# verdurin/pbdagcon

Hardware: AMD Instinct MI355X
Metric: consensus bases/sec (whole node) (higher is better)
Workload: dtype u8

## Files before the change

### pbdagcon_amd/csrc/api_run.hip.h

```cpp
namespace {

#define DQ_KMAX 52u
struct DgPlanIn { uint32_t T; uint64_t n_alns, sum_bb; uint32_t gcuts, max_segments, min_segment_len, seg_env, merge_q; };
struct DgPlan { uint32_t seg_max, seg_min, use_q, bp_max; };
static DgPlan dg_plan_pieces(const DgPlanIn &in) {
    DgPlan pl;
    const uint32_t T = in.T;
    pl.seg_min = in.min_segment_len;
    if (!pl.seg_min) pl.seg_min = (uint32_t)std::min<uint64_t>(768, std::max<uint64_t>(192, in.sum_bb / 8192));
    if (in.max_segments) pl.seg_max = in.max_segments > 64u ? 64u : in.max_segments;
    else if (in.seg_env) pl.seg_max = in.seg_env;
    else if (in.gcuts) pl.seg_max = 64;
    else { uint32_t sm = T ? 8192u / T : 8u; pl.seg_max = sm < 8u ? 8u : sm > 256u ? 256u : sm; }
    if (in.gcuts && !in.min_segment_len) pl.seg_min = 256;
    pl.use_q = 0;
    if (in.merge_q && !in.gcuts && pl.seg_max != 1) {
        const uint32_t slots = 1024u * DQ_WAVES;
        if (in.max_segments || in.seg_env) pl.use_q = 1;
        else if (T && in.n_alns <= (uint64_t)DQ_KMAX * T) {
            const uint64_t avail = std::min<uint64_t>(256, std::max<uint64_t>(1, in.sum_bb / T / 128));
            const uint64_t k = (uint64_t)T * avail / DQ_ROWS / slots;
            if (k >= 1 || (uint64_t)T * avail / DQ_ROWS * 10u >= 6u * slots) {
                const uint64_t sm = std::min<uint64_t>(avail, std::max<uint64_t>(k, 1) * slots * DQ_ROWS / T);
                if (sm >= 2) { pl.seg_max = (uint32_t)sm; pl.use_q = 1; }
// ... 130 lines not shown
    p.q_kmax = c->use_q && !c->opts.max_segments && !c->seg_env && c->max_k > DQ_KMAX ? DQ_KMAX : 0u;
    p.bp_seg_min = (c->seg_min + 2u) / 3u;
    p.seg_max = c->seg_max; p.seg_min = c->seg_min; p.cuts = c->run.cuts.as<uint32_t>(); p.bp_max = c->bp_max; p.cuts_bp = c->run.cuts_bp.as<uint32_t>(); p.bp_stat = c->run.bp_stat.as<float>(); p.bp_len = c->run.bp_len.as<uint32_t>();
    p.gcuts = c->gcuts; p.sh_log = c->sh_log;
    p.rd_s = c->run.rd.as<uint32_t>(); p.rd_e = p.rd_s + c->A; p.rd_lead = p.rd_e + c->A; p.rd_trail = p.rd_lead + c->A;
    p.pro_state = c->run.pro_state.as<uint32_t>(); p.sh_cnt = c->run.sh_cnt.as<uint32_t>();
    p.queue0 = c->run.queue0.as<int32_t>(); p.bp_end = c->run.bp_end.as<uint32_t>(); p.bp_ab = c->run.bp_ab.as<float>();
    p.defer = c->run.defer.as<uint32_t>(); p.cns_tmp0 = c->run.cns_tmp0.as<uint8_t>();
    p.seg_done = c->run.seg_done.as<uint32_t>(); p.wl_first = c->run.wl_first.as<uint32_t>();
    p.worklist = c->run.worklist.as<uint32_t>(); p.worklist_cap = c->worklist_cap;
    p.cns = c->run.cns.as<uint8_t>(); p.cns_cap = c->cns_cap;
    p.cns_off = c->sb.d<uint64_t>(c->sb.o_cns_off); p.cns_len = c->sb.d<uint32_t>(c->sb.o_cns_len);
    p.seg_first = c->sb.d<uint64_t>(c->sb.o_seg_first); p.n_seg = c->sb.d<uint32_t>(c->sb.o_n_seg);
    p.seg_r0 = c->run.seg.as<int32_t>(); p.seg_r1 = p.seg_r0 + seg_stride(c);
    p.seg_cap = c->seg_cap;
    p.st = c->sb.d<DgStatus>(0);
    if (c->opts.flags & DAGCON_FLAG_BASE_SUPPORT) {
        p.sup_tmp = c->run.sup_tmp.as<uint32_t>(); p.sup_tmp0 = c->run.sup_tmp0.as<uint32_t>();
        p.sup_w = c->run.sup.as<uint16_t>(); p.sup_d = p.sup_w + c->cns_cap;
    }
    if (c->opts.flags & DAGCON_FLAG_BASE_POS) {
        p.pos_tmp = c->run.pos_tmp.as<uint32_t>(); p.pos_tmp0 = c->run.pos_tmp0.as<uint32_t>(); p.pos_out = c->run.pos.as<uint32_t>();
    }
    if (c->ed_batch) {
        p.ed_seg = c->run.ed_seg.as<DgEdSeg>(); p.ed_out = c->run.ed_out.as<DgEdit>(); p.ed_cap = c->ed_cap;
        p.ed_top = c->sb.d<unsigned long long>(c->sb.o_ed_top);
        p.ed_t = c->cg.t.as<const uint8_t>(); p.ed_tbase = c->in.ed_tbase.as<const uint64_t>();
        if (c->evid_batch) p.evid = c->run.evid.as<DgEvid>();
    }
}

void launch_normalize(Ctx *c, const DgParams &p, const bool wide) {
    hipStream_t s = c->stream;
    if (c->A == 0) return;
    (void)hipMemsetAsync(c->run.ckpt.p, 0xFF, c->n_ckpt * 4, s);
    hipLaunchKernelGGL((k_norm_chunk<DG_NW, 64, false>), dim3((c->n_chunks + 63) / 64), dim3(64), 0, s, p);
    hipLaunchKernelGGL((k_norm_chunk<DG_NW_BIG, 32, true>), dim3((c->n_chunks + 31) / 32), dim3(32), 0, s, p);
    hipLaunchKernelGGL(k_norm_scan, dim3((c->A + 63) / 64), dim3(64), 0, s, p);
    if (wide) {
        hipLaunchKernelGGL(k_norm_finish2<uint32_t>, dim3((c->n_chunks + 3) / 4), dim3(256), 0, s, p);
        hipLaunchKernelGGL(k_normalize_slow<uint32_t>, dim3((c->A + 63) / 64), dim3(64), 0, s, p);
    } else {
        hipLaunchKernelGGL(k_norm_finish2<uint8_t>, dim3((c->n_chunks + 3) / 4), dim3(256), 0, s, p);
        hipLaunchKernelGGL(k_normalize_slow<uint8_t>, dim3((c->A + 63) / 64), dim3(64), 0, s, p);
    }
}

int launch_all(Ctx *c) {
    int r = ensure_arenas(c);
    if (r != DAGCON_OK) return r;
    DgParams p;
    fill_params(c, p);
    hipStream_t s = c->stream;
    const bool wide = matc_wide(c);
    if (c->poison & 8) {
        for (DevBuf *b : c->run.all())
            if (b->p && b->cap) HIPCHK(c, hipMemsetAsync(b->p, 0xEE, b->cap, s));
        if (c->sb.bytes > c->sb.zero_bytes) HIPCHK(c, hipMemsetAsync(c->sb.d<char>(c->sb.zero_bytes), 0xEE, c->sb.bytes - c->sb.zero_bytes, s));
    }
    HIPCHK(c, hipMemsetAsync(c->sb.dev.p, 0, c->sb.zero_bytes, s));
    if (c->matc_cells) HIPCHK(c, hipMemsetAsync(c->arena.matC.p, 0, matc_bytes(c), s));
    if (c->poison) {
        if ((c->poison & 1) && c->arena.matA.p) { HIPCHK(c, hipMemsetAsync(c->arena.matA.p, 0xEE, c->arena.matA.cap, s)); HIPCHK(c, hipMemsetAsync(c->arena.matD.p, 0xEE, c->arena.matD.cap, s)); }
        if ((c->poison & 2) && c->arena.nodes.p) { HIPCHK(c, hipMemsetAsync(c->arena.nodes.p, 0xEE, c->arena.nodes.cap, s)); HIPCHK(c, hipMemsetAsync(c->arena.pool.p, 0xEE, c->arena.pool.cap, s)); }
        if ((c->poison & 4) && c->arena.score_b.p) HIPCHK(c, hipMemsetAsync(c->arena.score_b.p, 0xEE, c->arena.score_b.cap, s));
        if ((c->poison & 4) && c->arena.norm.p) HIPCHK(c, hipMemsetAsync(c->arena.norm.p, 0xEE, c->arena.norm.cap, s));
    }
    HIPCHK(c, hipEventRecord(c->ev[0], s));
    launch_normalize(c, p, wide);
    HIPCHK(c, hipEventRecord(c->ev[1], s));
    hipLaunchKernelGGL(k_carve, dim3(1), dim3(1024), 0, s, p);
    if (c->T > 0) {
        const uint32_t rows4 = (c->max_tlen + 2 + 4 * DG_LPW - 1) / (4 * DG_LPW);
        if (c->gcuts && c->A > 0) hipLaunchKernelGGL(k_readspan, dim3((c->A + 63) / 64), dim3(64), 0, s, p);
        if (p.emit_scan && wide) hipLaunchKernelGGL(k_gsum<uint32_t>, dim3(c->T, (c->max_tlen + 2 + 255) / 256), dim3(256), 0, s, p);
        else if (p.emit_scan) hipLaunchKernelGGL(k_gsum<uint8_t>, dim3(c->T, (c->max_tlen + 2 + 1023) / 1024), dim3(256), 0, s, p);
        else hipLaunchKernelGGL(k_groups, dim3(c->T, (c->max_tlen + 2 + 31) / 32), dim3(256), 0, s, p);
        hipLaunchKernelGGL(k_gscan, dim3(c->T), dim3(1024), 0, s, p);
        if (c->A > 0) {
            const dim3 eg(c->T, (c->max_k + DG_ERPW - 1) / DG_ERPW, ((c->max_tlen + 2) >> c->emit_shift) + 1);
            if (wide) hipLaunchKernelGGL(k_emit<uint32_t>, eg, dim3(64), 0, s, p);
            else hipLaunchKernelGGL(k_emit<uint8_t>, eg, dim3(64), 0, s, p);
        }
        const size_t lds = (size_t)4 * 2 * (c->max_k + 2) * sizeof(int32_t);
        if (lds > 65536)
            HIPCHK(c, hipFuncSetAttribute((const void *)k_lists, hipFuncAttributeMaxDynamicSharedMemorySize, (int)lds));
        hipLaunchKernelGGL(k_lists, dim3(c->T, rows4), dim3(256), lds, s, p);
    }
    HIPCHK(c, hipEventRecord(c->ev[2], s));
    if (c->T > 0 && !(c->opts.flags & DAGCON_FLAG_STOP_AFTER_BUILD)) {
        if (c->gcuts) {
            HIPCHK(c, hipMemsetAsync(c->run.worklist.p, 0, 16, s));
            HIPCHK(c, hipMemsetAsync(c->run.seg_done.p, 0, (size_t)c->worklist_cap * (DG_SH_MAX + 1) * 4, s));
            hipLaunchKernelGGL(k_merge_pro, dim3(c->T), dim3(64), 0, s, p);
            hipLaunchKernelGGL(k_cuts2, dim3(c->T), dim3(64), 0, s, p);
            hipLaunchKernelGGL(k_merge_list, dim3(c->list_grid), dim3(64), 0, s, p);
            hipLaunchKernelGGL(k_merge_fin, dim3(c->T), dim3(64), 0, s, p);
        } else {
            hipLaunchKernelGGL(k_cuts, dim3(c->T), dim3(64), 0, s, p);
            if (c->use_q) {
                hipLaunchKernelGGL(k_merge_q, dim3((c->T * c->seg_max + DQ_ROWS - 1u) / DQ_ROWS), dim3(64), 0, s, p);
                if (p.q_kmax) hipLaunchKernelGGL(k_merge, dim3(c->T * c->seg_max), dim3(64), 0, s, p);
            } else hipLaunchKernelGGL(k_merge, dim3(c->T * c->seg_max), dim3(64), 0, s, p);
        }
    }
    HIPCHK(c, hipEventRecord(c->ev[3], s));
    if (c->T > 0 && !(c->opts.flags & (DAGCON_FLAG_STOP_AFTER_BUILD | DAGCON_FLAG_STOP_AFTER_MERGE))) {
        const bool sup = (c->opts.flags & DAGCON_FLAG_BASE_SUPPORT) != 0;
        const bool pos = (c->opts.flags & DAGCON_FLAG_BASE_POS) != 0;
#define DG_BP_LAUNCH(K, GRID)                                                                          \
        do {                                                                                           \
            if (sup && pos) hipLaunchKernelGGL((K<true, true>), GRID, dim3(64), 0, s, p);              \
            else if (sup) hipLaunchKernelGGL((K<true, false>), GRID, dim3(64), 0, s, p);               \
            else if (pos) hipLaunchKernelGGL((K<false, true>), GRID, dim3(64), 0, s, p);               \
            else hipLaunchKernelGGL((K<false, false>), GRID, dim3(64), 0, s, p);                       \
        } while (0)
        hipLaunchKernelGGL(k_bp_terms, dim3(c->T, 16), dim3(256), 0, s, p);
        if (c->gcuts) {
            hipLaunchKernelGGL(k_bp_xtree, dim3(c->T), dim3(64), 0, s, p);
            hipLaunchKernelGGL(k_bp_sweep_ab, dim3(c->T * c->bp_max), dim3(64), 0, s, p);
            hipLaunchKernelGGL(k_bp_comb, dim3(c->T), dim3(64), 0, s, p);
            hipLaunchKernelGGL(k_bp_abs, dim3(c->T * c->bp_max), dim3(256), 0, s, p);
            hipLaunchKernelGGL(k_bp_choose, dim3(c->T * c->bp_max), dim3(256), 0, s, p);
            hipLaunchKernelGGL(k_bp_sweep_abs_g, dim3(c->T * c->bp_max), dim3(64), 0, s, p);
            hipLaunchKernelGGL(k_bp_defer, dim3(c->T), dim3(64), 0, s, p);
            DG_BP_LAUNCH(k_bp_walk_g, dim3(c->T * c->bp_max));
        } else {
            if (p.bp_lane) hipLaunchKernelGGL(k_bp_sweep_l, dim3((c->T * c->bp_max + 7u) / 8u), dim3(64), 0, s, p);
            hipLaunchKernelGGL(k_bp_sweep, dim3(c->T * c->bp_max), dim3(64), 0, s, p);
            hipLaunchKernelGGL(k_bp_check, dim3(c->T), dim3(64), 0, s, p);
            if (p.bp_lane) DG_BP_LAUNCH(k_bp_walk_r, dim3((c->T * c->bp_max + 7u) / 8u));
            else DG_BP_LAUNCH(k_bp_walk, dim3(c->T * c->bp_max));
        }
        DG_BP_LAUNCH(k_bp_join, dim3(c->T));
#undef DG_BP_LAUNCH
        if (c->ed_batch) {
            const dim3 eg((uint32_t)((c->seg_cap + 3) / 4));
            hipLaunchKernelGGL(k_ed_scan_seg<false>, eg, dim3(256), 0, s, p);
            hipLaunchKernelGGL(k_ed_scan, dim3(1), dim3(1024), 0, s, p);
            hipLaunchKernelGGL(k_ed_scan_seg<true>, eg, dim3(256), 0, s, p);
            if (c->evid_batch) {
                hipLaunchKernelGGL(k_ev_windows, eg, dim3(256), 0, s, p);
                if (c->A > 0) hipLaunchKernelGGL(k_ev_count, dim3((c->A + 3) / 4), dim3(256), 0, s, p);
                hipLaunchKernelGGL(k_ev_spread, eg, dim3(256), 0, s, p);
            }
        }
    }
    HIPCHK(c, hipEventRecord(c->ev[4], s));
    HIPCHK(c, hipGetLastError());
    return DAGCON_OK;
}

}

extern "C" {

int dagcon_abi_version(void) { return DAGCON_ABI_VERSION; }

void dagcon_default_opts(dagcon_opts *o) {
    if (!o) return;
    memset(o, 0, sizeof *o);
    o->min_cov = 6; o->min_len = 500; o->trim = 50; o->min_weight = -1; o->device = 0; o->flags = 0;
}

const char *dagcon_last_error(const dagcon_ctx *ctx) {
    return ctx ? reinterpret_cast<const Ctx *>(ctx)->err.c_str() : "null context";
}

int dagcon_create(const dagcon_opts *opts, dagcon_ctx **out) {
    if (!opts || !out) return DAGCON_ERR_INVALID_ARG;
// ... 625 lines not shown
```

### pbdagcon_amd/csrc/k_build.hip.h

```cpp
#pragma once
#include <hip/hip_runtime.h>
#include "dagcon_dev.h"
#include "k_norm_run.hip.h"

#define DG_WAVE 64
#ifndef DG_LPW
#define DG_LPW 8u
#endif

__device__ __forceinline__ bool dg_failed(const DgParams &p) {
    return __hip_atomic_load(&p.st->err_flags, __ATOMIC_RELAXED, __HIP_MEMORY_SCOPE_AGENT) != 0;
}
__device__ __forceinline__ void dg_fail(const DgParams &p, uint32_t bit) {
    atomicOr(&p.st->err_flags, bit);
}
__device__ __forceinline__ void dg_fail_target(const DgParams &p, uint32_t t, uint32_t bit) {
    atomicOr(&p.tfail[t], bit);
}
__device__ __forceinline__ bool dg_tskip(const DgParams &p, uint32_t t) {
    return !p.tactive[t] || __hip_atomic_load(&p.tfail[t], __ATOMIC_RELAXED, __HIP_MEMORY_SCOPE_AGENT) != 0;
}
__device__ __forceinline__ bool dg_askip(const DgParams &p, uint32_t a) {
    return !(p.flags & DG_F_A1_ONLY) && __hip_atomic_load(&p.tfail[p.aln_tgt[a]], __ATOMIC_RELAXED, __HIP_MEMORY_SCOPE_AGENT) != 0;
}
// ... 810 lines not shown
                    const uint8_t qb = DG_Q(c), tb = DG_T(c);
                    if (qb == tb) {
                        const uint32_t cur = bidv[j];
                        acell[j] = ((uint32_t)tb << 25) | (prev + 1u);
                        if (f_anc_ok && kacc != 0u && kacc < (1u << 24)) f_key = kacc | ((pos - f_apos) << 24);
                        DG_DEPART(cur);
                        prev = cur; prev_pos = bbpos; fl = DG_EF_BB | DG_EF_OWN;
                    } else {
                        acell[j] = ((uint32_t)tb << 25) | DG_CELL_DEL;
                    }
                    bbpos++;
                    i++;
                }
            }
            if (p.fold) {
                const unsigned long long em = __ballot(f_key != 0u);
                if (em & (em - 1ull)) {
                    uint32_t fn;
                    const uint32_t vic = dg_emit_fold(em, f_key, f_first, pos, ndt, pool, &fn, lane);
                    if (vic | fn) {
                        const uint32_t dv = vic ? 0u : (f_first + 1u) | ((fn - 1u) << 25);
                        if (f_apos >= pos0) s_D[(f_apos - pos0) * 64 + lane] = dv;
                        if (f_apos < pos0 || f_apos == 0u) DG_ECELL(Dm, f_apos) = dv;
                        if (vic) acell[j] = (acell[j] & 0xFE000000u) | DG_CELL_DUP;
                    }
                }
            }
        }
        if (r < K && lane < DG_ERPW) {
#pragma unroll
            for (int j = 0; j < DG_EB; j++) {
                const uint32_t pos = pos0 + j;
                if (pos <= blen && pos >= P0 && pos < P1) {
                    DG_ECELL(Am, pos) = acell[j];
                    const uint32_t dv = s_D[j * 64 + lane];
                    if (pos > 0 || dv) DG_ECELL(Dm, pos) = dv;
                }
            }
            if (exit_val) DG_ECELL(Am, exitpos) = exit_val;
        }
        pos0 += DG_EB;
    }
    {
        const bool ahead = bbpos != DG_EDONE && (fl & DG_EF_OWN);
        uint32_t q = bbpos, nxt = 0;
        bool found = false, pfx_next = false;
        if (ahead) {
            while (i < hi) {
                const uint16_t c = buf[i];
                const uint8_t qb = DG_Q(c), tb = DG_T(c);
                if (qb == tb) { nxt = bid[q]; found = true; break; }
                if (qb == DG_GAP) { q++; i++; continue; }
                if (tb == DG_GAP) {
                    if (p.emit_scan) pfx_next = true; else nxt = gbase[q] + Cm[q];
                    found = true; break;
                }
                i++;
            }
        }
        if (p.emit_scan) {
            for (unsigned long long m = __ballot(pfx_next); m; m = __ballot(pfx_next)) {
                const uint32_t pp = (uint32_t)__builtin_amdgcn_readlane((int)q, __ffsll((long long)m) - 1);
                const uint32_t x = rvalid ? Cm[pp] : 0u;
                const uint32_t e = dg_wave_excl(x, lane);
                if (pfx_next && q == pp) { nxt = gbase[pp] + e; pfx_next = false; }
            }
        }
        if (ahead) {
            if (!found) {
                nxt = bid[exitpos];
                Am[(uint64_t)exitpos * K + r] = prev + 1u;
            }
            const uint32_t pos0 = 0xFFFFFFFFu;
            DG_DEPART(nxt);
        }
    }
#undef DG_EPW
#undef DG_ECELL
#undef DG_DEPART
#undef DG_COLUMN
#undef DG_STAGE
}

__device__ __forceinline__ int dg_lds_find(volatile int32_t *vals, int n, int x, int lane) {
    for (int b = 0; b < n; b += DG_WAVE) {
        int i = b + lane;
        bool hit = (i < n) && (vals[i] == x);
        unsigned long long m = __ballot(hit);
        if (m) return b + (__ffsll((long long)m) - 1);
    }
    return -1;
}

__device__ __forceinline__ uint32_t dg_pool_alloc(const DgParams &p, uint32_t t, uint32_t words, int lane) {
    uint32_t off = 0;
    if (lane == 0) {
        t = (uint32_t)__builtin_amdgcn_readfirstlane((int)t);
        off = atomicAdd(&p.pool_top[t], words);
        if ((uint64_t)off + words > p.pool_size[t]) { dg_fail(p, DG_E_POOL_TGT); p.st->bad_target = t; off = 0xFFFFFFFFu; }
    }
    return (uint32_t)__builtin_amdgcn_readlane((int)off, 0);
}

__device__ __forceinline__ unsigned long long dg_list_row(int32_t val, int32_t extra, int32_t chain, int32_t ulo, int32_t uhi,
                                                          int lane, int32_t &cnt, unsigned long long &cm) {
    cm = __ballot(val == chain);
    const bool uniq = val >= ulo && val < uhi;
    unsigned long long firsts = __ballot(uniq);
    cnt = 1 + extra;
    unsigned long long rem = __ballot(val != 0 && !uniq) & ~cm;
    while (rem) {
        const int first = __ffsll((long long)rem) - 1;
        const int32_t x = __builtin_amdgcn_readlane(val, first);
        const unsigned long long same = __ballot(val == x);
        rem &= ~same;
        if (lane == first) cnt = __popcll(same) + extra;
        firsts |= 1ull << first;
    }
    return firsts;
}

__device__ __forceinline__ void dg_lists_wave(const DgParams &p, uint32_t t, uint32_t pos0, uint32_t blen, uint32_t K,
                                              int lane) {
    const uint32_t npos = min(DG_LPW, blen + 2 - pos0);
    const uint64_t nb = p.node_base[t];
    const uint64_t bv = p.bbv_base[t];
    const uint32_t capb = dg_capb(K);
    const uint32_t fixed0 = 3u * p.t_nins[t];
    uint32_t *pool = p.pool + p.pool_base[t];
#define DG_LPOOL(OFF) (*reinterpret_cast<uint32_t *>(reinterpret_cast<char *>(pool) + (((uint32_t)(OFF)) << 2)))
    const uint32_t qb = pos0 - 1u + (uint32_t)lane;
    const uint32_t bidl = (lane < (int)DG_LPW + 2 && qb <= blen + 1) ? p.bid[bv + qb] : 0u;
    const uint32_t gbl = (lane <= (int)DG_LPW && pos0 + lane <= blen + 1) ? p.gbase[bv + pos0 + lane] : 0u;
    const uint32_t rb = (uint32_t)lane << 2;
    const bool rl = (uint32_t)lane < K;
    const uint32_t *Ar = p.matA + p.mat_base[t] + (uint64_t)pos0 * K, *Dr = p.matD + p.mat_base[t] + (uint64_t)pos0 * K;
#define DG_LROW(R) (rl ? *reinterpret_cast<const uint32_t *>(reinterpret_cast<const char *>(R) + rb) : 0u)
    uint32_t dcell = DG_LROW(Dr), acell = DG_LROW(Ar);
    const uint32_t lpos = pos0 + (uint32_t)lane;
    uint32_t r_lens = 0;
    uint32_t r_cov = 0;
    uint32_t r_out = fixed0 + lpos * 3u * capb, r_in = r_out + 2u * capb;
    uint32_t r_caps = capb | capb << 16;
    uint32_t pi = 0;
    for (; pi < npos; pi++) {
        const uint32_t pos = pos0 + pi;
        const uint32_t dep = dcell, arr = acell;
        if (pi + 1 < npos) {
            Ar += K; Dr += K;
            dcell = DG_LROW(Dr); acell = DG_LROW(Ar);
        }
        const bool mine = (uint32_t)lane == pi;
        const int32_t v1 = __builtin_amdgcn_readlane((int)bidl, pi + 1) + 1;
        uint32_t out_len = 0, in_len = 0;
        if (pos <= blen) {
            const int32_t val = (int32_t)DG_CELL_ID(dep), extra = (int32_t)(dep >> 25);
            const int32_t chain = __builtin_amdgcn_readlane((int)bidl, pi + 2) + 1;
            const int32_t ulo = __builtin_amdgcn_readlane((int)gbl, pi + 1) + 1;
            int32_t cnt;
            unsigned long long cm;
            const unsigned long long firsts = dg_list_row(val, extra, chain, ulo, chain, lane, cnt, cm);
            const uint32_t n = 1u + (uint32_t)__popcll(firsts);
            uint32_t off = fixed0 + pos * 3u * capb;
            if (n > capb) {
                const uint32_t cap = n + 2u;
                off = dg_pool_alloc(p, t, 2u * cap, lane);
                if (off == 0xFFFFFFFFu) break;
                if (mine) { r_out = off; r_caps = (r_caps & 0xFFFF0000u) | cap; }
            }
            const uint32_t idx = 1u + (uint32_t)__popcll(firsts & ((1ull << lane) - 1ull));
            if (lane == 0) { DG_LPOOL(off) = (uint32_t)(chain - 1); DG_LPOOL(off + 1) = (uint32_t)__popcll(cm); }
            if ((firsts >> lane) & 1ull) { DG_LPOOL(off + 2 * idx) = (uint32_t)(val - 1); DG_LPOOL(off + 2 * idx + 1) = (uint32_t)cnt; }
            out_len = n;
        }
        if (pos >= 1) {
            const uint32_t idf = DG_CELL_ID(arr);
            if (pos <= blen) {
                const unsigned long long covered = __ballot(arr != 0u);
                const uint32_t n_cov = (uint32_t)__popcll(covered);
                const uint32_t n_match = (uint32_t)__popcll(__ballot(arr != 0u && idf != DG_CELL_DEL));
                const uint32_t last_base = covered ? DG_CELL_BASE((uint32_t)__builtin_amdgcn_readlane((int)arr, 63 - __clzll((long long)covered))) : 0u;
                if (mine) r_cov = n_cov | n_match << 8 | last_base << 16;
            }
            const int32_t val = (arr != 0u && idf != DG_CELL_DEL && idf != DG_CELL_DUP) ? (int32_t)idf : 0;
            const int32_t chain = __builtin_amdgcn_readlane((int)bidl, pi) + 1;
            const int32_t ulo = __builtin_amdgcn_readlane((int)gbl, pi) + 1;
            int32_t cnt;
            unsigned long long cm;
            const unsigned long long firsts = dg_list_row(val, 0, chain, ulo, v1, lane, cnt, cm);
            const uint32_t n = 1u + (uint32_t)__popcll(firsts);
            uint32_t off = fixed0 + pos * 3u * capb + 2u * capb;
            if (n > capb) {
                const uint32_t cap = n + 2u;
                off = dg_pool_alloc(p, t, cap, lane);
                if (off == 0xFFFFFFFFu) break;
                if (mine) { r_in = off; r_caps = (r_caps & 0xFFFFu) | cap << 16; }
            }
            const uint32_t idx = 1u + (uint32_t)__popcll(firsts & ((1ull << lane) - 1ull));
            if (lane == 0) DG_LPOOL(off) = (uint32_t)(chain - 1);
            if ((firsts >> lane) & 1ull) DG_LPOOL(off + idx) = (uint32_t)(val - 1);
            in_len = n;
        }
        if (mine) r_lens = out_len | in_len << 16;
    }
    const uint32_t v = __shfl_down(bidl, 1);
    if ((uint32_t)lane < pi) {
        const bool inner = lpos >= 1 && lpos <= blen;
        const uint32_t n_cov = r_cov & 0xFFu, n_match = (r_cov >> 8) & 0xFFu;
        uint32_t base;
        if (lpos == 0) base = '^';
        else if (lpos == blen + 1) base = '$';
        else if (n_cov) base = r_cov >> 16;
        else base = p.bb ? p.bb[p.bb_off[t] + (lpos - 1)] : (uint8_t)'N';
        uint4 *rec = reinterpret_cast<uint4 *>(p.nodes + nb + v);
        rec[0] = make_uint4(r_lens, base | DG_NF_BACKBONE << 8,
                            inner ? 1u + n_match : 0u,
                            r_lens >> 16);
        rec[1] = make_uint4(r_out, r_in, r_caps, inner ? lpos : 0u);
        p.cov[bv + lpos] = inner ? (int32_t)n_cov : 0;
    }
#undef DG_LROW
#undef DG_LPOOL
}

__global__ __launch_bounds__(256) void k_lists(DgParams p) {
    extern __shared__ int32_t s_tmp[];
    const uint32_t t = blockIdx.x;
    if (dg_failed(p) || dg_tskip(p, t)) return;
    const int lane = threadIdx.x & 63, wave = threadIdx.x >> 6;
    const uint32_t blen = p.tlen[t];
    const uint32_t K = (uint32_t)(p.aln_begin[t + 1] - p.aln_begin[t]);
    if (K > DG_WAVE) {
    const uint32_t stride = p.max_k + 2;
    volatile int32_t *vals = s_tmp + (size_t)wave * 2 * stride;
    volatile int32_t *cnts = vals + stride;
    const uint64_t nb = p.node_base[t];
    const uint64_t bv = p.bbv_base[t];
    uint32_t *pool = p.pool + p.pool_base[t];
    const uint32_t *Am0 = p.matA + p.mat_base[t], *Dm0 = p.matD + p.mat_base[t];
    const uint32_t capb = dg_capb(K);
    const uint32_t fixed0 = 3u * p.t_nins[t];
    for (uint32_t pi = 0; pi < DG_LPW; pi++) {
    const uint32_t pos = (blockIdx.y * 4 + wave) * DG_LPW + pi;
    if (pos >= blen + 2) return;
    const uint32_t v = p.bid[bv + pos];
    const uint32_t *Am = Am0 + (uint64_t)pos * K;
    const uint32_t *Dm = Dm0 + (uint64_t)pos * K;
    const uint32_t fixed = fixed0 + pos * 3u * capb;
    uint32_t out_off = fixed, in_off = fixed + 2u * capb;
    uint32_t out_cap = capb, in_cap = capb;
    uint32_t out_len = 0, in_len = 0;
    uint32_t n_match = 0, n_cov = 0, last_base = 0;

    for (int dir = 0; dir < 2; dir++) {
        if (dir == 0 && pos == blen + 1) continue;
        if (dir == 1 && pos == 0) continue;
        const uint32_t *row = dir == 0 ? Dm : Am;
        int n = 1;
        int32_t lv = dir == 0 ? (int32_t)p.bid[bv + pos + 1] : (int32_t)p.bid[bv + pos - 1];
        int32_t lc = 0;
        bool in_lds = false;
        for (uint32_t r0 = 0; r0 < K; r0 += DG_WAVE) {
            const uint32_t r = r0 + lane;
            const uint32_t cell = r < K ? row[r] : 0u;
            int32_t val = (int32_t)DG_CELL_ID(cell);
            const int32_t extra = dir == 0 ? (int32_t)(cell >> 25) : 0;
            if (dir == 1) {
                const uint32_t idf = DG_CELL_ID(cell);
                const unsigned long long covered = __ballot(cell != 0u);
                if (pos <= blen) {
                    n_cov += (uint32_t)__popcll(covered);
                    n_match += (uint32_t)__popcll(__ballot(cell != 0u && idf != DG_CELL_DEL));
                    if (covered) last_base = DG_CELL_BASE((uint32_t)__builtin_amdgcn_readlane((int)cell, 63 - __clzll((long long)covered)));
                }
                val = (cell != 0u && idf != DG_CELL_DEL && idf != DG_CELL_DUP) ? (int32_t)idf : 0;
            }
            unsigned long long rem = __ballot(val != 0);
            if (!in_lds) {
                const int32_t chain = __builtin_amdgcn_readlane(lv, 0) + 1;
                const unsigned long long cm = __ballot(val == chain);
                if (lane == 0) lc += __popcll(cm);
                rem &= ~cm;
            }
            while (rem) {
                const int first = __ffsll((long long)rem) - 1;
                const int32_t x = __builtin_amdgcn_readlane(val, first);
                const unsigned long long same = __ballot(val == x);
                rem &= ~same;
                const int c = __popcll(same) + __builtin_amdgcn_readlane(extra, first);
                if (!in_lds) {
                    const unsigned long long hit = __ballot(lane < n && lv == x - 1);
                    if (hit) {
                        if (lane == __ffsll((long long)hit) - 1) lc += c;
                    } else if (n < DG_WAVE) {
                        if (lane == n) { lv = x - 1; lc = c; }
                        n++;
                    } else {
                        vals[lane] = lv; cnts[lane] = lc;
                        in_lds = true;
                    }
                }
                if (in_lds) {
                    const int idx = dg_lds_find(vals, n, x - 1, lane);
                    if (idx >= 0) {
                        if (lane == 0) cnts[idx] += c;
                    } else {
                        if (lane == 0) { vals[n] = x - 1; cnts[n] = c; }
                        n++;
                    }
                }
            }
        }
        if (n > 65000) { if (lane == 0) dg_fail_target(p, t, DG_E_INTERNAL); return; }
        uint32_t off = dir == 0 ? out_off : in_off;
        if ((uint32_t)n > capb) {
            const uint32_t cap = (uint32_t)n + 2u;
            off = dg_pool_alloc(p, t, dir == 0 ? 2u * cap : cap, lane);
            if (off == 0xFFFFFFFFu) return;
            if (dir == 0) { out_off = off; out_cap = cap; } else { in_off = off; in_cap = cap; }
        }
        if (!in_lds) {
            if (lane < n) {
                if (dir == 0) { pool[off + 2 * lane] = (uint32_t)lv; pool[off + 2 * lane + 1] = (uint32_t)lc; }
                else pool[off + lane] = (uint32_t)lv;
            }
        } else {
            for (int i = lane; i < n; i += DG_WAVE) {
                if (dir == 0) { pool[off + 2 * i] = (uint32_t)vals[i]; pool[off + 2 * i + 1] = (uint32_t)cnts[i]; }
                else pool[off + i] = (uint32_t)vals[i];
            }
        }
        if (dir == 0) out_len = (uint32_t)n; else in_len = (uint32_t)n;
    }
    if (lane == 0) {
        const bool inner = pos >= 1 && pos <= blen;
        DgNode nd;
        nd.out_len = (uint16_t)out_len;
        nd.in_len = (uint16_t)in_len;
        nd.flags = DG_NF_BACKBONE; nd.pad = 0;
        if (pos == 0) nd.base = '^';
        else if (pos == blen + 1) nd.base = '$';
        else if (n_cov) nd.base = (uint8_t)last_base;
        else nd.base = p.bb ? p.bb[p.bb_off[t] + (pos - 1)] : (uint8_t)'N';
        nd.weight = inner ? 1 + (int32_t)n_match : 0;
        nd.pending = (int32_t)in_len;
        nd.out_off = out_off; nd.in_off = in_off;
        nd.out_cap = (uint16_t)out_cap; nd.in_cap = (uint16_t)in_cap;
        nd.bbpos = inner ? (int32_t)pos : 0;
        p.cov[bv + pos] = inner ? (int32_t)n_cov : 0;
        p.nodes[nb + v] = nd;
    }
    }
    return;
    }
    const uint32_t pos0 = (blockIdx.y * 4 + (uint32_t)__builtin_amdgcn_readfirstlane(wave)) * DG_LPW;
    if (pos0 < blen + 2) dg_lists_wave(p, t, pos0, blen, K, lane);
}
```

Baseline: 359.7 million.

## Build backbone node lists one position per lane with LDS-staged rows

Replaces the wave-per-position list builder for targets with at most 64 alignments with a new kernel where each lane handles one backbone position. It stages the departure and arrival matrix rows into LDS, dedups them with a small per-lane table of non-unique IDs, and falls back to the old wave-cooperative path only for rows that overflow that table. The goal is to remove the serial per-position loop of ballots and readlanes. The cost is more LDS use, per-lane divergent scans over K cells, and an extra launch, with k_lists now only launched when max_k exceeds 64.

```diff
diff --git a/pbdagcon_amd/csrc/api_run.hip.h b/pbdagcon_amd/csrc/api_run.hip.h
--- a/pbdagcon_amd/csrc/api_run.hip.h
+++ b/pbdagcon_amd/csrc/api_run.hip.h
@@ -236,10 +236,15 @@
             if (wide) hipLaunchKernelGGL(k_emit<uint32_t>, eg, dim3(64), 0, s, p);
             else hipLaunchKernelGGL(k_emit<uint8_t>, eg, dim3(64), 0, s, p);
         }
-        const size_t lds = (size_t)4 * 2 * (c->max_k + 2) * sizeof(int32_t);
-        if (lds > 65536)
-            HIPCHK(c, hipFuncSetAttribute((const void *)k_lists, hipFuncAttributeMaxDynamicSharedMemorySize, (int)lds));
-        hipLaunchKernelGGL(k_lists, dim3(c->T, rows4), dim3(256), lds, s, p);
+        const size_t lds_lanes = (size_t)DG_LL_WAVES * DG_WAVE * (std::min<uint32_t>(c->max_k, DG_WAVE) | 1u) * sizeof(uint32_t);
+        hipLaunchKernelGGL(k_lists_lanes, dim3(c->T, (c->max_tlen + 2 + DG_LL_WAVES * DG_WAVE - 1) / (DG_LL_WAVES * DG_WAVE)),
+                           dim3(DG_LL_WAVES * DG_WAVE), lds_lanes, s, p);
+        if (c->max_k > DG_WAVE) {
+            const size_t lds = (size_t)4 * 2 * (c->max_k + 2) * sizeof(int32_t);
+            if (lds > 65536)
+                HIPCHK(c, hipFuncSetAttribute((const void *)k_lists, hipFuncAttributeMaxDynamicSharedMemorySize, (int)lds));
+            hipLaunchKernelGGL(k_lists, dim3(c->T, rows4), dim3(256), lds, s, p);
+        }
     }
     HIPCHK(c, hipEventRecord(c->ev[2], s));
     if (c->T > 0 && !(c->opts.flags & DAGCON_FLAG_STOP_AFTER_BUILD)) {
diff --git a/pbdagcon_amd/csrc/k_build.hip.h b/pbdagcon_amd/csrc/k_build.hip.h
--- a/pbdagcon_amd/csrc/k_build.hip.h
+++ b/pbdagcon_amd/csrc/k_build.hip.h
@@ -916,6 +916,7 @@
 #undef DG_STAGE
 }
 
+#include "k_lists_row.hip.h"
 __device__ __forceinline__ int dg_lds_find(volatile int32_t *vals, int n, int x, int lane) {
     for (int b = 0; b < n; b += DG_WAVE) {
         int i = b + lane;
@@ -954,107 +955,193 @@
     return firsts;
 }
 
-__device__ __forceinline__ void dg_lists_wave(const DgParams &p, uint32_t t, uint32_t pos0, uint32_t blen, uint32_t K,
+struct DgPosLists { uint32_t o_len, o_off, o_cap, i_len, i_off, i_cap, cov; };
+
+__device__ __forceinline__ bool dg_lists_pos(const DgParams &p, uint32_t t, uint32_t *pool, uint32_t pos, uint32_t blen,
+                                             uint32_t capb, uint32_t fixed0, int lane, bool do_out, bool do_in,
+                                             uint32_t dep, uint32_t arr, int32_t v1, int32_t chain_o, int32_t ulo_o,
+                                             int32_t chain_i, int32_t ulo_i, DgPosLists &r) {
+#define DG_LPOOL(OFF) (*reinterpret_cast<uint32_t *>(reinterpret_cast<char *>(pool) + (((uint32_t)(OFF)) << 2)))
+    if (do_out) {
+        const int32_t val = (int32_t)DG_CELL_ID(dep), extra = (int32_t)(dep >> 25);
+        int32_t cnt;
+        unsigned long long cm;
+        const unsigned long long firsts = dg_list_row(val, extra, chain_o, ulo_o, chain_o, lane, cnt, cm);
+        const uint32_t n = 1u + (uint32_t)__popcll(firsts);
+        uint32_t off = fixed0 + pos * 3u * capb, cap = capb;
+        if (n > capb) {
+            cap = n + 2u;
+            off = dg_pool_alloc(p, t, 2u * cap, lane);
+            if (off == 0xFFFFFFFFu) return false;
+        }
+        const uint32_t idx = 1u + (uint32_t)__popcll(firsts & ((1ull << lane) - 1ull));
+        if (lane == 0) { DG_LPOOL(off) = (uint32_t)(chain_o - 1); DG_LPOOL(off + 1) = (uint32_t)__popcll(cm); }
+        if ((firsts >> lane) & 1ull) { DG_LPOOL(off + 2 * idx) = (uint32_t)(val - 1); DG_LPOOL(off + 2 * idx + 1) = (uint32_t)cnt; }
+        r.o_len = n; r.o_off = off; r.o_cap = cap;
+    }
+    if (do_in) {
+        const uint32_t idf = DG_CELL_ID(arr);
+        r.cov = 0;
+        if (pos <= blen) {
+            const unsigned long long covered = __ballot(arr != 0u);
+            const uint32_t n_cov = (uint32_t)__popcll(covered);
+            const uint32_t n_match = (uint32_t)__popcll(__ballot(arr != 0u && idf != DG_CELL_DEL));
+            const uint32_t last_base = covered ? DG_CELL_BASE((uint32_t)__builtin_amdgcn_readlane((int)arr, 63 - __clzll((long long)covered))) : 0u;
+            r.cov = n_cov | n_match << 8 | last_base << 16;
+        }
+        const int32_t val = (arr != 0u && idf != DG_CELL_DEL && idf != DG_CELL_DUP) ? (int32_t)idf : 0;
+        int32_t cnt;
+        unsigned long long cm;
+        const unsigned long long firsts = dg_list_row(val, 0, chain_i, ulo_i, v1, lane, cnt, cm);
+        const uint32_t n = 1u + (uint32_t)__popcll(firsts);
+        uint32_t off = fixed0 + pos * 3u * capb + 2u * capb, cap = capb;
+        if (n > capb) {
+            cap = n + 2u;
+            off = dg_pool_alloc(p, t, cap, lane);
+            if (off == 0xFFFFFFFFu) return false;
+        }
+        const uint32_t idx = 1u + (uint32_t)__popcll(firsts & ((1ull << lane) - 1ull));
+        if (lane == 0) DG_LPOOL(off) = (uint32_t)(chain_i - 1);
+        if ((firsts >> lane) & 1ull) DG_LPOOL(off + idx) = (uint32_t)(val - 1);
+        r.i_len = n; r.i_off = off; r.i_cap = cap;
+    }
+#undef DG_LPOOL
+    return true;
+}
+
+__device__ __forceinline__ uint32_t dg_pool_alloc_lane(const DgParams &p, uint32_t t, uint32_t words) {
+    const uint32_t off = atomicAdd(&p.pool_top[t], words);
+    if ((uint64_t)off + words > p.pool_size[t]) { dg_fail(p, DG_E_POOL_TGT); p.st->bad_target = t; return 0xFFFFFFFFu; }
+    return off;
+}
+
+__device__ __forceinline__ void dg_stage_rows(uint32_t *rows, const uint32_t *blk, uint32_t nrows, uint32_t K, uint32_t S,
                                               int lane) {
-    const uint32_t npos = min(DG_LPW, blen + 2 - pos0);
+    if (K == 0) return;
+    const uint32_t total = nrows * K, q = DG_WAVE / K, rm = DG_WAVE % K;
+    uint32_t row = (uint32_t)lane / K, col = (uint32_t)lane % K;
+#pragma unroll 4
+    for (uint32_t i = (uint32_t)lane; i < total; i += DG_WAVE) {
+        rows[row * S + col] = blk[i];
+        row += q; col += rm;
+        if (col >= K) { col -= K; row++; }
+    }
+}
+
+#define DG_LL_WAVES 2u
+
+__global__ __launch_bounds__(64 * DG_LL_WAVES) void k_lists_lanes(DgParams p) {
+    extern __shared__ uint32_t s_rows[];
+    const uint32_t t = blockIdx.x;
+    if (dg_failed(p) || dg_tskip(p, t)) return;
+    const uint32_t K = (uint32_t)(p.aln_begin[t + 1] - p.aln_begin[t]);
+    if (K > DG_WAVE) return;
+    const uint32_t blen = p.tlen[t];
+    const int lane = threadIdx.x & 63;
+    const uint32_t wave = (uint32_t)__builtin_amdgcn_readfirstlane((int)(threadIdx.x >> 6));
+    const uint32_t pos0 = (blockIdx.y * DG_LL_WAVES + wave) * DG_WAVE;
+    if (pos0 >= blen + 2) return;
+    const uint32_t nrows = min((uint32_t)DG_WAVE, blen + 2 - pos0);
+    const uint32_t S = K | 1u;
+    uint32_t *rows = s_rows + wave * DG_WAVE * (min(p.max_k, (uint32_t)DG_WAVE) | 1u);
+    uint32_t *row = rows + (uint32_t)lane * S;
     const uint64_t nb = p.node_base[t];
     const uint64_t bv = p.bbv_base[t];
     const uint32_t capb = dg_capb(K);
     const uint32_t fixed0 = 3u * p.t_nins[t];
     uint32_t *pool = p.pool + p.pool_base[t];
-#define DG_LPOOL(OFF) (*reinterpret_cast<uint32_t *>(reinterpret_cast<char *>(pool) + (((uint32_t)(OFF)) << 2)))
-    const uint32_t qb = pos0 - 1u + (uint32_t)lane;
-    const uint32_t bidl = (lane < (int)DG_LPW + 2 && qb <= blen + 1) ? p.bid[bv + qb] : 0u;
-    const uint32_t gbl = (lane <= (int)DG_LPW && pos0 + lane <= blen + 1) ? p.gbase[bv + pos0 + lane] : 0u;
-    const uint32_t rb = (uint32_t)lane << 2;
-    const bool rl = (uint32_t)lane < K;
-    const uint32_t *Ar = p.matA + p.mat_base[t] + (uint64_t)pos0 * K, *Dr = p.matD + p.mat_base[t] + (uint64_t)pos0 * K;
-#define DG_LROW(R) (rl ? *reinterpret_cast<const uint32_t *>(reinterpret_cast<const char *>(R) + rb) : 0u)
-    uint32_t dcell = DG_LROW(Dr), acell = DG_LROW(Ar);
-    const uint32_t lpos = pos0 + (uint32_t)lane;
-    uint32_t r_lens = 0;
-    uint32_t r_cov = 0;
-    uint32_t r_out = fixed0 + lpos * 3u * capb, r_in = r_out + 2u * capb;
-    uint32_t r_caps = capb | capb << 16;
-    uint32_t pi = 0;
-    for (; pi < npos; pi++) {
-        const uint32_t pos = pos0 + pi;
-        const uint32_t dep = dcell, arr = acell;
-        if (pi + 1 < npos) {
-            Ar += K; Dr += K;
-            dcell = DG_LROW(Dr); acell = DG_LROW(Ar);
-        }
-        const bool mine = (uint32_t)lane == pi;
-        const int32_t v1 = __builtin_amdgcn_readlane((int)bidl, pi + 1) + 1;
-        uint32_t out_len = 0, in_len = 0;
-        if (pos <= blen) {
-            const int32_t val = (int32_t)DG_CELL_ID(dep), extra = (int32_t)(dep >> 25);
-            const int32_t chain = __builtin_amdgcn_readlane((int)bidl, pi + 2) + 1;
-            const int32_t ulo = __builtin_amdgcn_readlane((int)gbl, pi + 1) + 1;
-            int32_t cnt;
-            unsigned long long cm;
-            const unsigned long long firsts = dg_list_row(val, extra, chain, ulo, chain, lane, cnt, cm);
-            const uint32_t n = 1u + (uint32_t)__popcll(firsts);
-            uint32_t off = fixed0 + pos * 3u * capb;
-            if (n > capb) {
-                const uint32_t cap = n + 2u;
-                off = dg_pool_alloc(p, t, 2u * cap, lane);
-                if (off == 0xFFFFFFFFu) break;
-                if (mine) { r_out = off; r_caps = (r_caps & 0xFFFF0000u) | cap; }
-            }
-            const uint32_t idx = 1u + (uint32_t)__popcll(firsts & ((1ull << lane) - 1ull));
-            if (lane == 0) { DG_LPOOL(off) = (uint32_t)(chain - 1); DG_LPOOL(off + 1) = (uint32_t)__popcll(cm); }
-            if ((firsts >> lane) & 1ull) { DG_LPOOL(off + 2 * idx) = (uint32_t)(val - 1); DG_LPOOL(off + 2 * idx + 1) = (uint32_t)cnt; }
-            out_len = n;
-        }
-        if (pos >= 1) {
-            const uint32_t idf = DG_CELL_ID(arr);
-            if (pos <= blen) {
-                const unsigned long long covered = __ballot(arr != 0u);
-                const uint32_t n_cov = (uint32_t)__popcll(covered);
-                const uint32_t n_match = (uint32_t)__popcll(__ballot(arr != 0u && idf != DG_CELL_DEL));
-                const uint32_t last_base = covered ? DG_CELL_BASE((uint32_t)__builtin_amdgcn_readlane((int)arr, 63 - __clzll((long long)covered))) : 0u;
-                if (mine) r_cov = n_cov | n_match << 8 | last_base << 16;
-            }
-            const int32_t val = (arr != 0u && idf != DG_CELL_DEL && idf != DG_CELL_DUP) ? (int32_t)idf : 0;
-            const int32_t chain = __builtin_amdgcn_readlane((int)bidl, pi) + 1;
-            const int32_t ulo = __builtin_amdgcn_readlane((int)gbl, pi) + 1;
-            int32_t cnt;
-            unsigned long long cm;
-            const unsigned long long firsts = dg_list_row(val, 0, chain, ulo, v1, lane, cnt, cm);
-            const uint32_t n = 1u + (uint32_t)__popcll(firsts);
-            uint32_t off = fixed0 + pos * 3u * capb + 2u * capb;
-            if (n > capb) {
-                const uint32_t cap = n + 2u;
-                off = dg_pool_alloc(p, t, cap, lane);
-                if (off == 0xFFFFFFFFu) break;
-                if (mine) { r_in = off; r_caps = (r_caps & 0xFFFFu) | cap << 16; }
-            }
-            const uint32_t idx = 1u + (uint32_t)__popcll(firsts & ((1ull << lane) - 1ull));
-            if (lane == 0) DG_LPOOL(off) = (uint32_t)(chain - 1);
-            if ((firsts >> lane) & 1ull) DG_LPOOL(off + idx) = (uint32_t)(val - 1);
-            in_len = n;
-        }
-        if (mine) r_lens = out_len | in_len << 16;
-    }
-    const uint32_t v = __shfl_down(bidl, 1);
-    if ((uint32_t)lane < pi) {
-        const bool inner = lpos >= 1 && lpos <= blen;
+    const uint32_t *Db = p.matD + p.mat_base[t] + (uint64_t)pos0 * K, *Ab = p.matA + p.mat_base[t] + (uint64_t)pos0 * K;
+
+    const uint32_t pos = pos0 + (uint32_t)lane;
+    const bool act = (uint32_t)lane < nrows;
+    const bool do_out = act && pos <= blen, do_in = act && pos >= 1;
+    const uint32_t b0 = act ? p.bid[bv + pos] : 0u;
+    const uint32_t bm = do_in ? p.bid[bv + pos - 1] : 0u;
+    const uint32_t bp = do_out ? p.bid[bv + pos + 1] : 0u;
+    const uint32_t g0 = act ? p.gbase[bv + pos] : 0u;
+    const uint32_t g1 = do_out ? p.gbase[bv + pos + 1] : 0u;
+    uint32_t out_len = 0, in_len = 0, r_cov = 0;
+    uint32_t r_out = fixed0 + pos * 3u * capb, r_in = r_out + 2u * capb;
+    uint32_t out_cap = capb, in_cap = capb;
+    bool dead = false;
+
+    dg_stage_rows(rows, Db, nrows, K, S, lane);
+    __builtin_amdgcn_fence(__ATOMIC_SEQ_CST, "workgroup");
+    DgLaneRow so = {};
+    if (do_out) {
+        so = dg_lane_row<false>(row, K, bp + 1u, g1 + 1u, bp + 1u);
+        if (!so.overflow) {
+            if (so.n > capb) {
+                const uint32_t off = dg_pool_alloc_lane(p, t, 2u * (so.n + 2u));
+                if (off == 0xFFFFFFFFu) dead = true;
+                else { r_out = off; out_cap = so.n + 2u; }
+            }
+            if (!dead) { pool[r_out] = bp; pool[r_out + 1u] = so.c0; out_len = so.n; }
+        }
+    }
+    for (uint32_t j = 1; __ballot(j < out_len) != 0ull; j++)
+        if (j < out_len) {
+            const uint32_t e = row[j - 1u];
+            pool[r_out + 2u * j] = DG_CELL_ID(e) - 1u;
+            pool[r_out + 2u * j + 1u] = dg_lane_count(so, e);
+        }
+    __builtin_amdgcn_fence(__ATOMIC_SEQ_CST, "workgroup");
+
+    dg_stage_rows(rows, Ab, nrows, K, S, lane);
+    __builtin_amdgcn_fence(__ATOMIC_SEQ_CST, "workgroup");
+    DgLaneRow si = {};
+    if (do_in) {
+        si = dg_lane_row<true>(row, K, bm + 1u, g0 + 1u, b0 + 1u);
+        if (pos <= blen) r_cov = si.n_cov | si.n_match << 8 | si.last_base << 16;
+        if (!si.overflow && !dead) {
+            if (si.n > capb) {
+                const uint32_t off = dg_pool_alloc_lane(p, t, si.n + 2u);
+                if (off == 0xFFFFFFFFu) dead = true;
+                else { r_in = off; in_cap = si.n + 2u; }
+            }
+            if (!dead) { pool[r_in] = bm; in_len = si.n; }
+        }
+    }
+    for (uint32_t j = 1; __ballot(j < in_len) != 0ull; j++)
+        if (j < in_len) pool[r_in + j] = DG_CELL_ID(row[j - 1u]) - 1u;
+
+    const unsigned long long redo_o = __ballot(do_out && so.overflow != 0u), redo_i = __ballot(do_in && si.overflow != 0u);
+    for (unsigned long long rem = redo_o | redo_i; rem; rem &= rem - 1ull) {
+        const int pi = __ffsll((long long)rem) - 1;
+        const bool ro = (redo_o >> pi) & 1ull, ri = (redo_i >> pi) & 1ull;
+        const bool rl = (uint32_t)lane < K;
+        const uint32_t dep = rl && ro ? Db[(uint32_t)pi * K + (uint32_t)lane] : 0u;
+        const uint32_t arr = rl && ri ? Ab[(uint32_t)pi * K + (uint32_t)lane] : 0u;
+        DgPosLists r;
+        const bool ok = dg_lists_pos(p, t, pool, pos0 + (uint32_t)pi, blen, capb, fixed0, lane, ro, ri, dep, arr,
+                                     __builtin_amdgcn_readlane((int)b0, pi) + 1,
+                                     __builtin_amdgcn_readlane((int)bp, pi) + 1, __builtin_amdgcn_readlane((int)g1, pi) + 1,
+                                     __builtin_amdgcn_readlane((int)bm, pi) + 1, __builtin_amdgcn_readlane((int)g0, pi) + 1, r);
+        if (lane == pi) {
+            if (!ok) dead = true;
+            else {
+                if (ro) { out_len = r.o_len; r_out = r.o_off; out_cap = r.o_cap; }
+                if (ri) { in_len = r.i_len; r_in = r.i_off; in_cap = r.i_cap; r_cov = r.cov; }
+            }
+        }
+        if (!ok) break;
+    }
+
+    if (act && !dead) {
+        const bool inner = pos >= 1 && pos <= blen;
         const uint32_t n_cov = r_cov & 0xFFu, n_match = (r_cov >> 8) & 0xFFu;
         uint32_t base;
-        if (lpos == 0) base = '^';
-        else if (lpos == blen + 1) base = '$';
+        if (pos == 0) base = '^';
+        else if (pos == blen + 1) base = '$';
         else if (n_cov) base = r_cov >> 16;
-        else base = p.bb ? p.bb[p.bb_off[t] + (lpos - 1)] : (uint8_t)'N';
-        uint4 *rec = reinterpret_cast<uint4 *>(p.nodes + nb + v);
-        rec[0] = make_uint4(r_lens, base | DG_NF_BACKBONE << 8,
+        else base = p.bb ? p.bb[p.bb_off[t] + (pos - 1)] : (uint8_t)'N';
+        uint4 *rec = reinterpret_cast<uint4 *>(p.nodes + nb + b0);
+        rec[0] = make_uint4(out_len | in_len << 16, base | DG_NF_BACKBONE << 8,
                             inner ? 1u + n_match : 0u,
-                            r_lens >> 16);
-        rec[1] = make_uint4(r_out, r_in, r_caps, inner ? lpos : 0u);
-        p.cov[bv + lpos] = inner ? (int32_t)n_cov : 0;
-    }
-#undef DG_LROW
-#undef DG_LPOOL
+                            in_len);
+        rec[1] = make_uint4(r_out, r_in, out_cap | in_cap << 16, inner ? pos : 0u);
+        p.cov[bv + pos] = inner ? (int32_t)n_cov : 0;
+    }
 }
 
 __global__ __launch_bounds__(256) void k_lists(DgParams p) {
@@ -1064,7 +1151,7 @@
     const int lane = threadIdx.x & 63, wave = threadIdx.x >> 6;
     const uint32_t blen = p.tlen[t];
     const uint32_t K = (uint32_t)(p.aln_begin[t + 1] - p.aln_begin[t]);
-    if (K > DG_WAVE) {
+    if (K <= DG_WAVE) return;
     const uint32_t stride = p.max_k + 2;
     volatile int32_t *vals = s_tmp + (size_t)wave * 2 * stride;
     volatile int32_t *cnts = vals + stride;
@@ -1185,8 +1272,4 @@
         p.nodes[nb + v] = nd;
     }
     }
-    return;
-    }
-    const uint32_t pos0 = (blockIdx.y * 4 + (uint32_t)__builtin_amdgcn_readfirstlane(wave)) * DG_LPW;
-    if (pos0 < blen + 2) dg_lists_wave(p, t, pos0, blen, K, lane);
-}
+}
diff --git a/pbdagcon_amd/csrc/k_lists_row.hip.h b/pbdagcon_amd/csrc/k_lists_row.hip.h
--- /dev/null
+++ b/pbdagcon_amd/csrc/k_lists_row.hip.h
@@ -0,0 +1,85 @@
+#pragma once
+#include <stdint.h>
+
+#ifndef DG_HD_INLINE
+#if defined(__HIPCC__)
+#include <hip/hip_runtime.h>
+#define DG_HD_INLINE __host__ __device__ __forceinline__
+#else
+#define DG_HD_INLINE inline __attribute__((always_inline))
+#endif
+#endif
+#ifndef DG_CELL_ID
+#define DG_CELL_ID(c)   ((c) & 0x1FFFFFFu)
+#define DG_CELL_DEL     0x1FFFFFFu
+#endif
+#ifndef DG_CELL_DUP
+#define DG_CELL_DUP 0x1FFFFFEu
+#endif
+
+#define DG_LTAB 4u
+
+struct DgLaneRow {
+    uint32_t n;
+    uint32_t c0;
+    uint32_t tv[DG_LTAB];
+    uint32_t tc[DG_LTAB];
+    uint32_t overflow;
+    uint32_t n_cov, n_match, last_base;
+};
+
+template <bool ARRIVAL>
+DG_HD_INLINE void dg_lane_cell(DgLaneRow &s, const uint32_t cell, uint32_t *row, const uint32_t chain,
+                               const uint32_t ulo, const uint32_t uspan) {
+    uint32_t val = DG_CELL_ID(cell);
+    if (ARRIVAL) {
+        s.n_cov += cell != 0u;
+        s.n_match += (cell != 0u) & (val != DG_CELL_DEL);
+        s.last_base = cell != 0u ? cell >> 25 : s.last_base;
+        val = ((val == DG_CELL_DEL) | (val == DG_CELL_DUP)) ? 0u : val;
+    }
+    s.c0 += val == chain;
+    const bool uniq = val - ulo < uspan;
+    bool newo = !uniq & (val != 0u) & (val != chain);
+#pragma unroll
+    for (uint32_t k = 0; k < DG_LTAB; k++) {
+        const bool h = s.tv[k] == val;
+        s.tc[k] += h;
+        newo &= !h;
+    }
+    s.overflow |= newo ? s.tv[DG_LTAB - 1u] : 0u;
+#pragma unroll
+    for (uint32_t k = DG_LTAB - 1u; k > 0; k--) {
+        s.tv[k] = newo ? s.tv[k - 1u] : s.tv[k];
+        s.tc[k] = newo ? s.tc[k - 1u] : s.tc[k];
+    }
+    s.tv[0] = newo ? val : s.tv[0];
+    s.tc[0] = newo ? 1u : s.tc[0];
+    if (uniq | newo) { row[s.n - 1u] = ARRIVAL ? val : cell; s.n++; }
+}
+
+template <bool ARRIVAL>
+DG_HD_INLINE DgLaneRow dg_lane_row(uint32_t *row, const uint32_t K, const uint32_t chain, const uint32_t ulo,
+                                   const uint32_t uhi) {
+    DgLaneRow s = {};
+    s.n = 1u;
+    const uint32_t uspan = uhi > ulo ? uhi - ulo : 0u;
+    uint32_t r = 0;
+    for (; r + 4u <= K; r += 4u) {
+        const uint32_t c0 = row[r], c1 = row[r + 1u], c2 = row[r + 2u], c3 = row[r + 3u];
+        dg_lane_cell<ARRIVAL>(s, c0, row, chain, ulo, uspan);
+        dg_lane_cell<ARRIVAL>(s, c1, row, chain, ulo, uspan);
+        dg_lane_cell<ARRIVAL>(s, c2, row, chain, ulo, uspan);
+        dg_lane_cell<ARRIVAL>(s, c3, row, chain, ulo, uspan);
+    }
+    for (; r < K; r++) dg_lane_cell<ARRIVAL>(s, row[r], row, chain, ulo, uspan);
+    return s;
+}
+
+DG_HD_INLINE uint32_t dg_lane_count(const DgLaneRow &s, const uint32_t e) {
+    const uint32_t id = DG_CELL_ID(e), extra = e >> 25;
+    uint32_t cnt = 1u;
+#pragma unroll
+    for (uint32_t k = 0; k < DG_LTAB; k++) cnt = s.tv[k] == id ? s.tc[k] : cnt;
+    return cnt + extra;
+}
```

New measurement: 367.0 million (median of 6 runs). Within noise of the previous version (+2.0%).
